# pymc-devs/pymc

Measured on AMD Instinct MI355X. Metric: effective samples/sec (and leapfrog steps/sec), 10k-param hierarchical logistic regression, one NUTS chain per GPU, higher is better.
Workload: dtype f64

## Files before the change

pymc_amd/csrc/engine.hip:

```cpp
#include <hip/hip_runtime.h>

#include <algorithm>
#include <atomic>
#include <chrono>
#include <cmath>
#include <cstdio>
#include <cstdlib>
#include <cstring>
#include <mutex>
#include <thread>
#include <utility>
#include <ctime>
#include <string>
#include <vector>

#include "kernels.h"
#include "small_kernel.h"
#include "mixture_kernel.h"
#include "nuts_mi355.h"
#include "pcg64_stream.h"
#include "advi.h"

static thread_local std::string g_err;

// ... 2049 lines not shown
  nuts_velocity_energy_fn hp_velocity_energy = nullptr;
  void* hp_user = nullptr;
  std::vector<double> hp_p, hp_v;
  double* kin_user_dev = nullptr;
  int full_adapt = 0, fa_mfma = 1;
  double *fa_L = nullptr, *fa_Lw = nullptr, *fa_fg_mean = nullptr, *fa_fg_raw = nullptr, *fa_bg_mean = nullptr, *fa_bg_raw = nullptr;
  double *fa_scratch = nullptr, *fa_rhs = nullptr;
  int *fa_fail = nullptr;
  double fa_fg_n = 0, fa_bg_n = 0;
  int64_t fa_previous_update = 0;
  std::vector<double> fa_initial_cov;
  double *wa_mean = nullptr, *wa_m2 = nullptr, *wb_mean = nullptr, *wb_m2 = nullptr;
  bool fg_is_a = true;
  double fg_count = 0, bg_count = 0;
  std::vector<double> initial_mean, initial_diag;
  int64_t n_samples = 0, adaptation_window = 101;
  bool window_switched = false;
  DualAvg da{};
  bool tune = true;
  int64_t iter_count = 0, divergences = 0;
  double step_size = 0;
  double* stage_dev = nullptr;
  double* stage_host = nullptr;
  double* out_dev = nullptr;
  double* out_dev2 = nullptr;
  bool small = false;
  int small_lds_slots = 0;
  int small_one_wave = 1;
  int group_wide = 0;
  double* out_host = nullptr;
  HostStatus* st_dev = nullptr;
  HostStatus* st_host = nullptr;
  int seq = 0;
  std::vector<double> div_source, div_dest;
  bool cache_ok = false;
  std::vector<double> last_q;
  double last_logp = 0.0;
  DrawOut* do_dev = nullptr;
  DrawOut* do_host = nullptr;
  DrawOutMapped* dom_host = nullptr;
  DrawOutMapped* dom_dev = nullptr;
  unsigned dom_seq = 0;
  double* kin_part = nullptr;
  int64_t cache_epoch = -1;
  int fold_ctl = 1;
  CtlJob pend{}; bool pend_valid = false;
  bool defer_last_ctl = false; int xfold = 1;
  int next_dir = 0; bool pre_done = false; int xpre = 1;
  bool edge_pair = false;
  ArenaDev shA{};
  EdgePlan ep;
  int spec_max = 10, last_depth = 0;
  int pipe_draws = 1;
  int logs_done = 0, logs_total = 0;
  double* many_in_host = nullptr; double* many_in_dev = nullptr; char* many_out_host = nullptr; char* many_out_dev = nullptr;
  size_t many_in_cap = 0, many_out_cap = 0;
  double t_begin = 0, t_loop = 0, t_wait = 0, t_finish = 0, t_post = 0;
  double tm_pre = 0, tm_start = 0, tm_tree = 0, tm_record = 0, tm_host = 0, tm_post = 0;
  int64_t tm_draws = 0, tm_batches = 0;
  int64_t leapfrogs = 0;
  int n_uni_cap = 0;
  template <typename T>
  T* keep(T* p) { owned.push_back((void*)p); return p; }
};

extern "C" void nuts_chain_config_default(nuts_chain_config* c) {
  std::memset(c, 0, sizeof(*c));
  c->step_scale = 0.25; c->Emax = 1000; c->target_accept = 0.8; c->gamma = 0.05; c->k = 0.75; c->t0 = 10;
  c->adapt_step_size = 1; c->max_treedepth = 10; c->early_max_treedepth = 8;
  c->potential = NUTS_POT_DIAG_ADAPT; c->initial_weight = 0; c->adaptation_window = 101; c->discard_window = 50;
  c->exp_alpha = 0.02; c->exp_stop_adaptation = INFINITY; c->exp_use_grads = 0;
  c->adaptation_window_multiplier = 1; c->early_update = 0;
}

static void fa_factor(nuts_chain* c, const double* raw, double denom) {
  const int n = c->n;
  hipStream_t s = c->m->stream;
  const dim3 g2((n + 255) / 256, n);
  hipLaunchKernelGGL(k_fa_cov, g2, dim3(256), 0, s, n, raw, denom, c->dense_C, c->fa_Lw, c->fa_fail);
  const int nb = (n + FA_NB - 1) / FA_NB;
  for (int k = 0; k < nb; ++k) {
    hipLaunchKernelGGL(k_chol_panel, dim3(nb - k), dim3(256), 0, s, n, c->fa_Lw, k, c->fa_fail);
    const int m = nb - k - 1;
    if (m > 0) hipLaunchKernelGGL(k_chol_update, dim3(m * (m + 1) / 2), dim3(256), 0, s, n, c->fa_Lw, k, nb, c->fa_mfma);
  }
  hipLaunchKernelGGL(k_fa_commit, dim3(1024), dim3(256), 0, s, (int64_t)n * n, c->fa_Lw, c->fa_L, c->fa_fail, c->fa_fail + 1);
}
static void fa_random(nuts_chain* c, const double* z_dev, double* p_out) {
  const int n = c->n;
  hipStream_t s = c->m->stream;
  hipMemcpyAsync(c->fa_rhs, z_dev, n * sizeof(double), hipMemcpyDeviceToDevice, s);
  const int nb = (n + FA_NB - 1) / FA_NB;
  for (int b = nb - 1; b >= 0; --b)
    hipLaunchKernelGGL(k_trsv_block, dim3(std::max(1, (b * FA_NB + 255) / 256)), dim3(256), 0, s, n, c->fa_L, c->fa_rhs, p_out, b);
}
static int fa_reset(nuts_chain* c) {
  const int n = c->n;
  const size_t nn = (size_t)n * n;
  const double w = c->cfg.initial_weight;
  std::vector<double> raw(nn);
  for (size_t e = 0; e < nn; ++e) raw[e] = c->fa_initial_cov[e] * w;
  HIPCHK(hipMemcpy(c->fa_fg_raw, raw.data(), nn * sizeof(double), hipMemcpyHostToDevice));
  HIPCHK(hipMemcpy(c->fa_fg_mean, c->initial_mean.data(), n * sizeof(double), hipMemcpyHostToDevice));
  HIPCHK(hipMemset(c->fa_bg_raw, 0, nn * sizeof(double)));
  HIPCHK(hipMemset(c->fa_bg_mean, 0, n * sizeof(double)));
  HIPCHK(hipMemset(c->fa_fail, 0, 2 * sizeof(int)));
// ... 51 lines not shown
    c->fg_count = w; c->bg_count = 0;
  }
  if (c->full_adapt) { const int rc = fa_reset(c); if (rc) return rc; }
  if (c->cfg.potential == NUTS_POT_DIAG_ADAPT_EXP) {
    HIPCHK(hipMemset(c->wa_mean, 0, n * sizeof(double))); HIPCHK(hipMemset(c->wa_m2, 0, n * sizeof(double)));
    HIPCHK(hipMemset(c->wb_mean, 0, n * sizeof(double))); HIPCHK(hipMemset(c->wb_m2, 0, n * sizeof(double)));
  }
  c->n_samples = 0;
  return NUTS_OK;
}

extern "C" nuts_chain* nuts_chain_create(nuts_model* m, const nuts_chain_config* cfg) {
  if (!m || !cfg) { g_err = "null argument"; return nullptr; }
  if (cfg->potential < NUTS_POT_DIAG_ADAPT || cfg->potential > NUTS_POT_HOST) { g_err = "unknown potential kind"; return nullptr;
  }
  if (cfg->potential == NUTS_POT_FULL && (!cfg->dense_cov || !cfg->dense_rand)) { g_err = "dense potential needs dense_cov and dense_rand"; return nullptr; }
  if (cfg->potential == NUTS_POT_FULL_ADAPT && !cfg->dense_cov) { g_err = "NUTS_POT_FULL_ADAPT needs dense_cov (the initial covariance)"; return nullptr; }
  if (cfg->max_treedepth < 1 || cfg->max_treedepth > MAX_LEVELS - 1) { g_err = "max_treedepth out of range (1..11)"; return nullptr; }
  if ((cfg->potential == NUTS_POT_FULL || cfg->potential == NUTS_POT_FULL_ADAPT || cfg->potential == NUTS_POT_HOST) && m->md.lg.ga) {
    g_err = "a dense mass matrix needs the span-partitioned row pass: create the model with NUTS_ROWS_NO_GROUP_ALIGNED";
    return nullptr;
  }
  auto* c = new nuts_chain();
  c->m = m; c->cfg = *cfg; c->n = m->md.n;
  m->n_chains++;
  const int n = c->n;
  c->initial_mean.assign(n, 0.0);
  c->initial_diag.assign(n, 1.0);
  if (cfg->initial_mean) c->initial_mean.assign(cfg->initial_mean, cfg->initial_mean + n);
  if (cfg->initial_diag) c->initial_diag.assign(cfg->initial_diag, cfg->initial_diag + n);
  else if (cfg->potential == NUTS_POT_DIAG_ADAPT) c->cfg.initial_weight = 1;
  c->cfg.initial_mean = nullptr; c->cfg.initial_diag = nullptr;
  c->host_pot = cfg->potential == NUTS_POT_HOST;
  c->dense = cfg->potential == NUTS_POT_FULL || cfg->potential == NUTS_POT_FULL_ADAPT || c->host_pot;
  c->full_adapt = cfg->potential == NUTS_POT_FULL_ADAPT;
  c->fa_mfma = env_int("NUTS_FA_MFMA", 1);
  if (c->cfg.fa_update_window < 1) c->cfg.fa_update_window = 1;
  if (c->dense) c->initial_diag.assign(m->md.n, 1.0);
  c->cfg.dense_cov = nullptr; c->cfg.dense_rand = nullptr;
  c->adaptation_window = cfg->adaptation_window;
  ArenaDev& A = c->A;
  A.n = n;
  const int maxd = std::max(cfg->max_treedepth, cfg->early_max_treedepth);
  A.S = 1 << maxd;
  A.ept = m->ept;
  A.nblk = m->md.nblk;
  const size_t arena = (size_t)A.S * n;
  A.Q = c->keep(dev_alloc<double>(arena)); A.P = c->keep(dev_alloc<double>(arena));
  A.V = c->keep(dev_alloc<double>(arena)); A.G = c->keep(dev_alloc<double>(arena));
  A.E = c->keep(dev_alloc<double>(A.S)); A.LOGP = c->keep(dev_alloc<double>(A.S));
  A.PS = c->keep(dev_alloc<double>((size_t)MAX_LEVELS * n));
  A.PSUM = c->keep(dev_alloc<double>(n));
  c->kin_part = c->keep(dev_alloc<double>((size_t)A.nblk));
  A.ctl = c->keep(dev_alloc<Ctl>(1));
  c->var = c->keep(dev_alloc<double>(n)); c->stds = c->keep(dev_alloc<double>(n)); c->inv_stds = c->keep(dev_alloc<double>(n));
  c->wa_mean = c->keep(dev_alloc<double>(n)); c->wa_m2 = c->keep(dev_alloc<double>(n));
  c->wb_mean = c->keep(dev_alloc<double>(n)); c->wb_m2 = c->keep(dev_alloc<double>(n));
  A.var = c->var; A.inv_stds = c->inv_stds;
  A.ga_ticket = m->md.lg.ga ? m->md.lg.ga_ticket : nullptr; A.ga_nticket = m->md.lg.ga ? 2 * m->md.lg.ga_nblk : 0;
  if (c->full_adapt) {
    const size_t nn = (size_t)n * n;
    c->fa_initial_cov.assign(cfg->dense_cov, cfg->dense_cov + nn);
    c->dense_C = c->keep(dev_alloc<double>(nn));
    c->fa_L = c->keep(dev_alloc<double>(nn)); c->fa_Lw = c->keep(dev_alloc<double>(nn));
    c->fa_fg_raw = c->keep(dev_alloc<double>(nn)); c->fa_bg_raw = c->keep(dev_alloc<double>(nn));
    c->fa_fg_mean = c->keep(dev_alloc<double>(n)); c->fa_bg_mean = c->keep(dev_alloc<double>(n));
    c->fa_scratch = c->keep(dev_alloc<double>(4 * (size_t)n)); c->fa_rhs = c->keep(dev_alloc<double>(n));
    c->fa_fail = c->keep(dev_alloc<int>(2));
    c->mv_grid = (n + (256 / WAVE) - 1) / (256 / WAVE);
  } else if (c->host_pot) {
    c->hp_p.assign(n, 0.0); c->hp_v.assign(n, 0.0);
    c->kin_user_dev = c->keep(dev_alloc<double>(1));
    A.kin_user = c->kin_user_dev;
  } else if (c->dense) {
    c->dense_C = c->keep(dev_upload(cfg->dense_cov, (size_t)n * n));
    c->dense_W = c->keep(dev_upload(cfg->dense_rand, (size_t)n * n));
    c->mv_grid = (n + (256 / WAVE) - 1) / (256 / WAVE);
  }
  c->n_uni_cap = (1 << maxd) + 2 * maxd + 16;
  c->stage_dev = c->keep(dev_alloc<double>(2 * (size_t)n + 2 * (size_t)c->n_uni_cap));
  c->out_dev = c->keep(dev_alloc<double>(2 * (size_t)n));
  c->out_dev2 = c->keep(dev_alloc<double>(2 * (size_t)n + 2));
  c->fold_ctl = env_int("NUTS_FOLD_CTL", 1) != 0 && !(m->md.has_mvn && m->md.mv.winv);
  c->spec_max = env_int("NUTS_SPEC_MAX", 10);
  c->xfold = env_int("NUTS_XFOLD", 1);
  c->edge_pair = m->ep_ok && env_int("NUTS_EDGE_PAIR", 1) != 0 && !c->dense && !c->host_pot && !m->md.has_mvn && !m->explicit_pre &&
                 m->md.lean_ok && c->fold_ctl && c->xfold;
  if (c->edge_pair) {
    c->shA = A;
    c->shA.S = 2;
    c->shA.Q = c->keep(dev_alloc<double>(2 * (size_t)n)); c->shA.P = c->keep(dev_alloc<double>(2 * (size_t)n));
    c->shA.V = c->keep(dev_alloc<double>(2 * (size_t)n)); c->shA.G = c->keep(dev_alloc<double>(2 * (size_t)n));
    if (!c->shA.Q || !c->shA.P || !c->shA.V || !c->shA.G) { (void)hipGetLastError(); c->edge_pair = false; }
    c->ep.ring = std::max(1, std::min(GA_RING_LEAVES, env_int("NUTS_EDGE_PAIR_RING", GA_RING_LEAVES)));
  }
  c->pipe_draws = env_int("NUTS_PIPE_DRAWS", 1) != 0;
  c->xpre = env_int("NUTS_XPRE", 1);
  c->small_lds_slots = env_int("NUTS_SMALL_LDS", 1) == 0 ? -1 : env_int("NUTS_SMALL_LDS_SLOTS", 0);
  c->small_one_wave = env_int("NUTS_SMALL_ONE_WAVE", 1);
  c->group_wide = env_int("NUTS_GROUP_WIDE", 0);
  const bool glm_small = m->md.has_glm && env_int("NUTS_GLM_SMALL", 1) != 0 && m->md.glm.Xt && !m->md.glm.beta_buf && m->md.glm.off_beta >= 0 && m->md.n_derived == 0 && n <= 256;
  c->small = env_int("NUTS_SMALL_KERNEL", 1) != 0 && n <= SMALL_MAX_N && m->ept == 1 && !m->md.has_logit && !m->md.has_mvn && !m->md.has_mix &&
             (!m->md.has_glm || glm_small) &&
             m->md.n_lins == 0 && m->factor_elems <= SMALL_MAX_ELEMS && !c->dense;
  c->do_dev = c->keep(dev_alloc<DrawOut>(1));
  A.uniforms = c->stage_dev + 2 * (size_t)n;
  A.log_uniforms = A.uniforms + c->n_uni_cap;
  for (void* p : c->owned)
    if (!p) { g_err = "device allocation failed (trajectory arena needs 4*2^max_treedepth*n*8 bytes)"; nuts_chain_destroy(c); return nullptr; }
  if (hipHostMalloc((void**)&c->stage_host, (2 * (size_t)n + 2 * (size_t)c->n_uni_cap) * sizeof(double), hipHostMallocDefault) != hipSuccess ||
      hipHostMalloc((void**)&c->out_host, 2 * (size_t)n * sizeof(double), hipHostMallocDefault) != hipSuccess ||
      hipHostMalloc((void**)&c->st_host, sizeof(HostStatus), hipHostMallocMapped) != hipSuccess ||
      hipHostGetDevicePointer((void**)&c->st_dev, c->st_host, 0) != hipSuccess ||
      hipHostMalloc((void**)&c->do_host, sizeof(DrawOut), hipHostMallocDefault) != hipSuccess ||
      hipHostMalloc((void**)&c->dom_host, DOM_RING * sizeof(DrawOutMapped), hipHostMallocMapped) != hipSuccess ||
      hipHostGetDevicePointer((void**)&c->dom_dev, c->dom_host, 0) != hipSuccess) {
    g_err = "pinned host allocation failed"; nuts_chain_destroy(c); return nullptr;
  }
  hipMemset(A.ctl, 0, sizeof(Ctl));
  std::memset(c->st_host, 0, sizeof(HostStatus));
  std::memset(c->dom_host, 0, DOM_RING * sizeof(DrawOutMapped));
  c->step_size = cfg->step_scale / std::pow((double)n, 0.25);
  c->da = DualAvg{c->step_size, cfg->target_accept, cfg->gamma, cfg->k, cfg->t0, 0, 0, 0, 0, 1};
  c->da.reset();
  if (potential_reset(c) != NUTS_OK) { nuts_chain_destroy(c); return nullptr; }
  return c;
}

extern "C" void nuts_chain_destroy(nuts_chain* c) {
  if (!c) return;
  if (c->m) hipStreamSynchronize(c->m->stream);
  if (c->m && c->m->group) group_remove_model(c->m->group, c->m);
  if (c->m) c->m->n_chains--;
  for (void* p : c->owned) if (p) hipFree(p);
  if (c->stage_host) hipHostFree(c->stage_host);
  if (c->out_host) hipHostFree(c->out_host);
  if (c->st_host) hipHostFree(c->st_host);
  if (c->do_host) hipHostFree(c->do_host);
  if (c->dom_host) hipHostFree(c->dom_host);
  if (c->many_in_host) hipHostFree(c->many_in_host);
  if (c->many_out_host) hipHostFree(c->many_out_host);
  if (c->many_in_dev) hipFree(c->many_in_dev);
  if (c->many_out_dev) hipFree(c->many_out_dev);
  delete c;
}

static void group_remove_model(nuts_group* g, nuts_model* m) {
  if (!g || !m || m->group != g) return;
  hipStreamSynchronize(g->stream);
  std::lock_guard<std::mutex> lk(g->mu);
  for (int i = 0; i < GRP_MAXC; ++i)
    if (g->member[i] == m) { g->member[i] = nullptr; g->n--; g->konst_set[i] = false; if (i < GAL_MAXC) g->gal_konst_set[i] = false; }
  if (m->g_active) { g->nactive--; m->g_active = false; }
  m->group = nullptr;
  m->stream = m->own_stream;
}

extern "C" nuts_group* nuts_group_create(void) {
  nuts_group* g = new nuts_group();
  if (hipStreamCreateWithFlags(&g->stream, hipStreamNonBlocking) != hipSuccess) { g_err = "nuts_group_create: no stream"; delete g; return nullptr; }
  return g;
}

extern "C" int nuts_group_add(nuts_group* g, nuts_chain* c) {
  if (!g || !c || !c->m) return NUTS_E_ARG;
  nuts_model* m = c->m;
  const MvnDev& mv = m->md.mv;
  if (m->group) { g_err = "nuts_group_add: the chain's model already belongs to a group"; return NUTS_E_ARG; }
  if (m->n_chains != 1) { g_err = "nuts_group_add: a member model carries exactly one chain (its launch parity and records are the chain's)"; return NUTS_E_ARG; }
  const RowsDev& lg = m->md.lg;
  const bool is_mvn = m->md.has_mvn && (mv.aligned == 4 || mv.aligned == 8);
  const bool is_rows = m->md.has_logit && !m->md.has_mvn && lg.ga && lg.ga_naux == 0 && lg.D == 8 && m->ga_struct_ok == 1;
// ... 424 lines not shown
  const int* abort_flag = mode == MODE_TREE ? &A.ctl->aborted : nullptr;
  const int t = gm.edge + gm.dir * (j + 1), src = gm.edge + gm.dir * j;
  const int64_t d_o = (int64_t)(t & (A.S - 1)) * A.n, so = (int64_t)(src & (A.S - 1)) * A.n;
  HostStatus* const st = mode == MODE_TREE ? c->st_dev : (HostStatus*)nullptr;
  io.lean = m->md.lean_ok && !c->dense && (!io.explicit_pre || m->md.n_deferred == 0);
  const bool foldable = c->fold_ctl && (mode == MODE_TREE || (mode == MODE_SIMPLE && n_simple > 0));
  const bool last = mode == MODE_TREE ? j + 1 == (1 << d) : j + 1 == n_simple;
  if (io.lean && foldable) {
    if (io.explicit_pre) {
      const bool al_xpre = m->md.mv.aligned && mode == MODE_TREE && c->xpre;
      if (j == 0 && !(al_xpre && c->pre_done)) hipLaunchKernelGGL(k_leaf_pre, dim3(A.nblk), dim3(VEC_THREADS), 0, s, A, io, j);
      if (j == 0) c->pre_done = false;
      io.pre_next = last ? 0 : 1;
      if (last && al_xpre && c->defer_last_ctl && c->next_dir != 0) {
        io.pre_next = c->next_dir == gm.dir ? 1 : 3;
        c->pre_done = true;
      }
    }
    const bool deferrable = (io.explicit_pre ? m->md.mv.aligned != 0 : m->md.lg.ga != 0) && mode == MODE_TREE;
    CtlJob* job = (deferrable && j == 0 && c->pend_valid) ? &c->pend : nullptr;
    if (job && !io.explicit_pre) job->src_prev = job->io.dir == io.dir;
    launch_dense(m, A, io, j, (j > 0 || job) ? 1 : 0, d, c->cfg.Emax, max_depth, st, job);
    if (job) c->pend_valid = false;
    launch_vector(m, A, io, j, d);
    if (last) {
      if (deferrable && c->defer_last_ctl) { c->pend = CtlJob{io, j, d, seq, false}; c->pend_valid = true; }
      else launch_control_lean(m, A, io, j, d, c->cfg.Emax, max_depth, st, seq);
    }
    c->leapfrogs++;
    return;
  }
  if (io.explicit_pre) hipLaunchKernelGGL(k_leaf_pre, dim3(A.nblk), dim3(VEC_THREADS), 0, s, A, io, j);
  if (c->dense)
    dense_velocity(c, A.P + d_o, A.V + d_o, A.Q + so, A.Q + d_o, gm.eps, abort_flag, VEL_ONLY);
  launch_dense(m, A, io, j, 0, d, c->cfg.Emax, max_depth, st);
  launch_vector(m, A, io, j, d);
  if (io.lean) launch_control_lean(m, A, io, j, d, c->cfg.Emax, max_depth, st, seq);
  else if (m->has_prog) hipLaunchKernelGGL(k_control<true>, dim3(1), dim3(VEC_THREADS), 0, s, m->md, A, io, j, d, c->cfg.Emax, max_depth, st, seq);
  else hipLaunchKernelGGL(k_control<false>, dim3(1), dim3(VEC_THREADS), 0, s, m->md, A, io, j, d, c->cfg.Emax, max_depth, st, seq);
  if (c->dense) {
    dense_velocity(c, A.P + d_o, A.V + d_o, nullptr, nullptr, 0.0, abort_flag, VEL_LEAF);
    const dim3 grid(m->md.nblk);
    switch (m->ept) {
      case 1: hipLaunchKernelGGL(k_tree_vec<1>, grid, dim3(VEC_THREADS), 0, s, m->md, A, io, j, d); break;
      case 4: hipLaunchKernelGGL(k_tree_vec<4>, grid, dim3(VEC_THREADS), 0, s, m->md, A, io, j, d); break;
      default: hipLaunchKernelGGL(k_tree_vec<16>, grid, dim3(VEC_THREADS), 0, s, m->md, A, io, j, d); break;
    }
    hipLaunchKernelGGL(k_tree_ctl, dim3(1), dim3(VEC_THREADS), 0, s, m->md, A, io, j, d, c->cfg.Emax, max_depth,
                       mode == MODE_TREE ? c->st_dev : (HostStatus*)nullptr, seq);
  }
  c->leapfrogs++;
}

static int run_tree(nuts_chain* c, const double* uniforms, double step_size, int max_depth, unsigned* flags_out, bool* exhausted_out,
                    int* cursor_out = nullptr) {
  int rc = NUTS_OK;
  bool exhausted = true;
  GroupTreeScope lockstep(c->dense || c->host_pot ? nullptr : c->m);
  unsigned flags = 0;
  Geometry gm{uniforms[0] < 0.5 ? 1 : -1, 0, 0, 0, 0.0};
  gm.eps = gm.dir > 0 ? step_size : -step_size;
  auto next_geometry = [&](const Geometry& g, int d, int dir) {
    Geometry r = g;
    if (g.dir > 0) r.right += 1 << d; else r.left -= 1 << d;
    r.dir = dir;
    r.edge = dir > 0 ? r.right : r.left;
    r.eps = dir > 0 ? step_size : -step_size;
    return r;
  };
  const int spec = c->host_pot ? 0 : std::min(c->spec_max, c->last_depth - 1);
  const bool pairing = c->edge_pair && !c->m->group && !c->host_pot && !c->dense;
  int turns = 0;
  int ep_replays_in[32] = {};
  int prev_dir = 0;
  bool ep_bad = false;
  c->ep.reset();
  c->m->ep_launch.kind = EP_PLAIN;
  auto enqueue_doubling = [&](const Geometry& g, int d) {
    const int nleaf = 1 << d;
    ensure_logs(c, (2 << d) + d + 1);
    const int seq = ++c->seq;
    c->defer_last_ctl = c->xfold && c->fold_ctl && d + 1 < max_depth && d + 1 <= spec;
    c->next_dir = c->defer_last_ctl ? (uniforms[(2 << d) + d] < 0.5 ? 1 : -1) : 0;
    if (pairing) c->ep.begin(d, g.dir, std::min(spec, max_depth - 1), [&](int e) { return uniforms[(1 << e) + e - 1] < 0.5 ? 1 : -1; });
    for (int j = 0; j < nleaf; ++j) {
      if (pairing) {
        nuts_model::EpLaunch& el = c->m->ep_launch;
        int k = 0;
        el.kind = c->ep.leaf(g.dir, &el.slot, &k);
        if (el.kind == EP_REPLAY) ++ep_replays_in[std::min(d, 31)];
        if (el.kind == EP_REPLAY && k != j) { g_err = "internal error: edge pairing replays a leaf out of order"; ep_bad = true; el.kind = EP_PLAIN; }
        if (el.kind == EP_PAIRED) {
          const int od = -g.dir;
          EvalIO sio{};
          sio.mode = MODE_SIMPLE; sio.lean = 1;
          sio.dir = od; sio.edge = od > 0 ? g.right : g.left; sio.left = g.left; sio.right = g.right;
          sio.eps = od > 0 ? step_size : -step_size;
          el.sio = sio; el.sj = k; el.sA = c->shA;
          el.first = k == 0;
          el.sfold = k > 0 ? GA_FOLD_SRC : (j == 0 && d > 0 && prev_dir == od ? GA_FOLD_SRC : 0);
        }
      }
      enqueue_leaf(c, g, j, d, MODE_TREE, max_depth, j + 1 == nleaf ? seq : 0);
    }
    prev_dir = g.dir;
    c->defer_last_ctl = false;
    return seq;
  };
  c->pre_done = false;
  c->pend_valid = false;
  auto flush_pending = [&](int seq_waited) {
    if (!c->pend_valid || c->pend.seq != seq_waited) return;
    const CtlJob& p = c->pend;
    launch_control_lean(c->m, c->A, p.io, p.j, p.d, c->cfg.Emax, max_depth, c->st_dev, p.seq);
    c->pend_valid = false;
  };
  Geometry ahead{};
  int ahead_seq = 0;
  int seq = enqueue_doubling(gm, 0);
  int depth_done = 0;
  for (int d = 0; d < max_depth; ++d) {
    if (d + 1 < max_depth && d + 1 <= spec) {
      ahead = next_geometry(gm, d, uniforms[(2 << d) + d] < 0.5 ? 1 : -1);
      ahead_seq = enqueue_doubling(ahead, d + 1);
    } else ahead_seq = 0;
    flush_pending(seq);
    if (c->cb_err) return host_pot_error(c);
    const auto tw0 = clk::now();
    rc = wait_status(c, seq, &flags, cursor_out);
    c->t_wait += secs(tw0, clk::now());
    if (rc) return rc;
    depth_done = d + 1;
    if (flags & ST_BAD_ENERGY) break;
    if (flags & (ST_DIVERGING | ST_TURNING)) { exhausted = false; break; }
    if (d + 1 >= max_depth) break;
    const int dir = (flags & ST_DIR_POS) ? 1 : -1;
    turns += dir != gm.dir;
    if (ahead_seq) {
      if (ahead.dir != dir) { g_err = "internal error: look-ahead mispredicted the direction of a doubling"; return NUTS_E_HIP; }
      gm = ahead; seq = ahead_seq;
    } else {
      gm = next_geometry(gm, d, dir);
      seq = enqueue_doubling(gm, d + 1);
    }
  }
  c->last_depth = depth_done;
  c->pend_valid = false;
  if (depth_done >= 4) c->m->ep_turns = std::max(c->m->ep_turns, turns);
  c->m->ep_ring_full = c->ep.ring_full;
  if (pairing) {
    c->m->ep_dropped += c->ep.n;
    for (int d = depth_done; d < 32; ++d) c->m->ep_dropped += ep_replays_in[d];
  }
  if (ep_bad) return NUTS_E_HIP;
  *flags_out = flags;
  *exhausted_out = exhausted;
  return NUTS_OK;
}

static void launch_small(nuts_chain* c, const ArenaDev& A, const SmallDrawArgs& a) {
#define SMALL_LAUNCH(NT, P) hipLaunchKernelGGL((k_small_draw<NT, P>), dim3(1), dim3(NT), 0, c->m->stream, c->m->md, A, a)
  const bool hp = c->m->has_prog;
  if (c->n <= WAVE && c->small_one_wave && !c->m->md.has_glm) { if (hp) SMALL_LAUNCH(64, true); else SMALL_LAUNCH(64, false); }
  else if (c->n <= 256) { if (hp) SMALL_LAUNCH(256, true); else SMALL_LAUNCH(256, false); }
  else if (c->n <= 512) { if (hp) SMALL_LAUNCH(512, true); else SMALL_LAUNCH(512, false); }
  else { if (hp) SMALL_LAUNCH(1024, true); else SMALL_LAUNCH(1024, false); }
#undef SMALL_LAUNCH
}

static int finish_draw_host(nuts_chain* c, const DrawOut& o, bool adapt, bool exhausted, const double* result_dev, int64_t evals,
                            double perf_start, double perf_diff, double cpu_diff, nuts_draw_stats* stats) {
  c->da.update(std::exp(o.log_accept_sum) / o.n_proposals, adapt);
  int rc = potential_update(c, result_dev, result_dev + c->n);
  if (rc) return rc;
  if (o.diverging) { rc = read_divergence_points(c, o.div_t); if (rc) return rc; }
  if (!c->tune) c->divergences += o.diverging != 0;
  c->iter_count += 1;
  fill_draw_stats(c, o, exhausted, evals, perf_start, perf_diff, cpu_diff, stats);
  return NUTS_OK;
}

static SmallDrawArgs small_draw_args(const nuts_chain* c, bool cached, const DrawPlan& plan) {
  SmallDrawArgs a{};
  a.q_src = cached ? c->out_dev2 : nullptr; a.g_src = cached ? c->out_dev2 + c->n : nullptr; a.cached_logp = c->last_logp;
  a.step_size = plan.step_size; a.Emax = c->cfg.Emax; a.max_depth = plan.max_depth;
  a.worst_uniforms = plan.need_uni;
  a.q_out = c->out_dev; a.g_out = c->out_dev + c->n; a.st = nullptr; a.seq = 0; a.lds_slots = c->small_lds_slots;
  return a;
}

static int draw_one_small(nuts_chain* c, const double* q0, const double* normals, const double* uniforms, const DrawPlan& plan,
                          bool* exhausted, const double** result_dev) {
  const int n = c->n;
  hipStream_t s = c->m->stream;
  ArenaDev& A = c->A;
  const bool cached = start_cached(c, q0);
  std::memcpy(c->stage_host, q0, n * sizeof(double));
  std::memcpy(c->stage_host + n, normals, n * sizeof(double));
  std::memcpy(c->stage_host + 2 * n, uniforms, plan.need_uni * sizeof(double));
  HIPCHK(hipMemcpyAsync(c->stage_dev, c->stage_host, (2 * (size_t)n + plan.need_uni) * sizeof(double), hipMemcpyHostToDevice, s));
  if (!cached) HIPCHK(hipMemcpyAsync(A.Q, c->stage_dev, n * sizeof(double), hipMemcpyDeviceToDevice, s));
  SmallDrawArgs a = small_draw_args(c, cached, plan);
  a.normals = c->stage_dev + n;
  a.n_draws = 1; a.n_uniforms = plan.need_uni;
  a.trace_q = nullptr; a.out = c->do_dev; a.n_done = nullptr;
  launch_small(c, A, a);
  std::swap(c->out_dev, c->out_dev2);
// ... 69 lines not shown
  double* const h_q = c->many_in_host;
  double* const h_norm = h_q + n;
  double* const h_u = h_norm + (size_t)K * n;
  double* const h_lu = h_u + U;
  std::memcpy(h_q, q0, n * sizeof(double));
  std::memcpy(h_norm, normals, (size_t)K * n * sizeof(double));
  std::memcpy(h_u, uniforms, U * sizeof(double));
  for (size_t i = 0; i < U; ++i) h_lu[i] = std::log(h_u[i]);
  HIPCHK(hipMemcpyAsync(c->many_in_dev, c->many_in_host, in_doubles * sizeof(double), hipMemcpyHostToDevice, s));
  const double* const d_norm = c->many_in_dev + n;
  const double* const d_u = d_norm + (size_t)K * n;
  const double* const d_lu = d_u + U;
  double* const trace_dev = reinterpret_cast<double*>(c->many_out_dev);
  if (!cached0) {
    HIPCHK(hipMemcpyAsync(A.Q, c->many_in_dev, n * sizeof(double), hipMemcpyDeviceToDevice, s));
    model_enqueue_plain(c->m, A.Q, A.G, A.LOGP);
  }
  const double* const save_u = A.uniforms; const double* const save_lu = A.log_uniforms;
  const int save_done = c->logs_done, save_total = c->logs_total;
  c->logs_done = c->logs_total = 1 << 30;
  int done = 0;
  size_t consumed = 0;
  const int fgrid = std::max(1, std::min(256, (n + VEC_THREADS - 1) / VEC_THREADS));
  c->tm_pre += secs(tm0, clk::now()); c->tm_batches++;
  const bool pipe = !c->tune && !c->full_adapt && c->pipe_draws;
  struct Pending {
    bool valid = false; int k = 0; unsigned seq = 0; bool exhausted = false, adapt = false; size_t consumed_after = 0; int cursor = 0;
    double perf_start = 0.0, wall = 0.0, cpu = 0.0;
  } pend;
  auto enqueue_start = [&](int k, const DrawPlan& plan, size_t at, bool from_prev) {
    A.uniforms = d_u + at; A.log_uniforms = d_lu + at;
    return enqueue_draw_start(c, d_norm + (size_t)k * n, false, from_prev, plan.step_size, 0, plan.max_depth, k > 0 ? (const DrawOut*)c->do_dev : nullptr);
  };
  auto complete = [&](const Pending& p, bool* diverged) -> int {
    const auto tb = clk::now();
    DrawOutMapped* slot = c->dom_host + (p.seq % DOM_RING);
    unsigned long long seen = 0;
    int r = wait_seq(c, &slot->seq, 0, p.seq, "k_draw_finish ended without publishing its record", &seen);
    if (r) return r;
    const DrawOut o = slot->o;
    const auto t1 = clk::now();
    c->tm_record += secs(tb, t1);
    if (o.cursor != p.cursor) { g_err = "internal error: the status word and the draw record disagree on the uniforms consumed"; return NUTS_E_HIP; }
    r = finish_draw_host(c, o, p.adapt, p.exhausted, c->out_dev, o.n_proposals + ((p.k == 0 && !cached0) ? 1 : 0), p.perf_start, p.wall, p.cpu,
                         stats + p.k);
    c->tm_host += secs(t1, clk::now()); c->tm_draws++;
    if (r) return r;
    stats[p.k].n_uniforms_consumed = (int32_t)p.consumed_after;
    c->last_logp = o.logp;
    done = p.k + 1;
    *diverged = o.diverging != 0;
    return NUTS_OK;
  };
  bool started = false;
  for (int k = 0; k < K; ++k) {
    const DrawClock dclock;
    const DrawPlan plan = plan_draw(c);
    const size_t need_uni = (size_t)plan.need_uni;
    if (!started) {
      if (U - consumed < need_uni) {
        if (k == 0) { g_err = "not enough uniforms for the worst-case tree"; rc = NUTS_E_ARG; }
        break;
      }
      rc = enqueue_start(k, plan, consumed, k > 0 || cached0);
      if (rc) break;
    }
    started = false;
    unsigned flags = 0;
    bool exhausted = true;
    int cursor = 0;
    const auto ta = clk::now();
    c->tm_start += secs(dclock.t0, ta);
    rc = run_tree(c, h_u + consumed, plan.step_size, plan.max_depth, &flags, &exhausted, &cursor);
    const auto tb = clk::now();
    c->tm_tree += secs(ta, tb);
    if (rc) break;
    if (flags & ST_BAD_ENERGY) {
      if (pend.valid) { bool dv = false; rc = complete(pend, &dv); pend.valid = false; if (rc) break; }
      rc = bad_initial_energy(c);
      break;
    }
    const unsigned seq = ++c->dom_seq;
    hipLaunchKernelGGL(k_draw_finish, dim3(fgrid), dim3(VEC_THREADS), 0, s, A, c->out_dev, c->out_dev + n, c->do_dev, trace_dev + (size_t)k * n,
                       c->dom_dev + (seq % DOM_RING), seq);
    const size_t consumed_after = consumed + (size_t)cursor;
    if (pipe && !(flags & ST_DIVERGING) && k + 1 < K && U - consumed_after >= need_uni) {
      rc = enqueue_start(k + 1, plan, consumed_after, true);
      if (rc) break;
      started = true;
    }
    Pending cur;
    cur.valid = true; cur.k = k; cur.seq = seq; cur.exhausted = exhausted; cur.adapt = plan.adapt; cur.consumed_after = consumed_after; cur.cursor = cursor;
    cur.perf_start = dclock.perf_start(); cur.wall = dclock.wall(); cur.cpu = dclock.cpu();
    bool diverged = false;
    if (pend.valid) { rc = complete(pend, &diverged); pend.valid = false; if (rc) break; }
    if (started) pend = cur;
    else { rc = complete(cur, &diverged); if (rc) break; }
    consumed = consumed_after;
    if (diverged) break;
  }
  if (pend.valid) {
    bool dv = false;
    const int r2 = complete(pend, &dv);
    pend.valid = false;
    if (!rc) rc = r2;
  }
  A.uniforms = save_u; A.log_uniforms = save_lu;
  c->logs_done = save_done; c->logs_total = save_total;
  *n_done = done;
  const auto tm1 = clk::now();
  struct PostTimer { nuts_chain* c; clk::time_point t; ~PostTimer() { c->tm_post += secs(t, clk::now()); } } post_timer{c, tm1};
  if (done > 0) {
    HIPCHK(hipMemcpyAsync(c->many_out_host, c->many_out_dev, (size_t)done * n * sizeof(double), hipMemcpyDeviceToHost, s));
    HIPCHK(hipStreamSynchronize(s));
    HIPCHK(hipGetLastError());
    const double* trace_host = reinterpret_cast<const double*>(c->many_out_host);
    std::memcpy(q_out, trace_host, (size_t)done * n * sizeof(double));
    commit_start_cache(c, trace_host + (size_t)(done - 1) * n, c->last_logp);
  } else {
    hipStreamSynchronize(s);
  }
  if (rc && done > 0 && rc != NUTS_E_BAD_ENERGY) return rc;
  return done > 0 ? NUTS_OK : (rc ? rc : NUTS_E_ARG);
}

extern "C" int nuts_chain_draw_many(nuts_chain* c, const double* q0, const double* normals, const double* uniforms,
                                    int32_t n_uniforms, int32_t K, double* q_out, nuts_draw_stats* stats, int32_t* n_done) {
  if (!c || !q0 || !normals || !uniforms || !q_out || !stats || !n_done || K <= 0) { g_err = "null argument"; return NUTS_E_ARG; }
  if (c->host_pot) { g_err = "nuts_chain_draw_many: a host potential is consulted between draws (random, update): one nuts_chain_draw per transition"; return NUTS_E_ARG; }
  if (!c->small) return draw_many_general(c, q0, normals, uniforms, n_uniforms, K, q_out, stats, n_done);
  if (c->tune) { g_err = "nuts_chain_draw_many: the chain is still tuning (the single-launch batch has no adaptation between its draws)"; return NUTS_E_ARG; }
  const DrawClock dclock;
  const int n = c->n;
  hipStream_t s = c->m->stream;
  ArenaDev& A = c->A;
  const DrawPlan plan = plan_draw(c);
  if (n_uniforms < plan.need_uni) { g_err = "not enough uniforms for the worst-case tree"; return NUTS_E_ARG; }
  const size_t in_doubles = (size_t)n + (size_t)K * n + (size_t)n_uniforms;
  const size_t trace_bytes = (size_t)K * n * sizeof(double), outs_bytes = (size_t)K * sizeof(DrawOut);
  const size_t out_bytes = trace_bytes + outs_bytes + 16;
  int rc = ensure_many_staging(c, in_doubles, out_bytes);
  if (rc) return rc;
  const bool cached = start_cached(c, q0);
  std::memcpy(c->many_in_host, q0, n * sizeof(double));
  std::memcpy(c->many_in_host + n, normals, (size_t)K * n * sizeof(double));
  std::memcpy(c->many_in_host + n + (size_t)K * n, uniforms, (size_t)n_uniforms * sizeof(double));
  HIPCHK(hipMemcpyAsync(c->many_in_dev, c->many_in_host, in_doubles * sizeof(double), hipMemcpyHostToDevice, s));
  if (!cached) HIPCHK(hipMemcpyAsync(A.Q, c->many_in_dev, n * sizeof(double), hipMemcpyDeviceToDevice, s));
  ArenaDev Am = A;
  Am.uniforms = c->many_in_dev + n + (size_t)K * n;
  SmallDrawArgs a = small_draw_args(c, cached, plan);
  a.normals = c->many_in_dev + n;
  a.n_draws = K; a.n_uniforms = n_uniforms;
  a.trace_q = reinterpret_cast<double*>(c->many_out_dev);
  a.out = reinterpret_cast<DrawOut*>(c->many_out_dev + trace_bytes);
  a.n_done = reinterpret_cast<int*>(c->many_out_dev + trace_bytes + outs_bytes);
  launch_small(c, Am, a);
// ... 135 lines not shown
  for (int k = 0; k < 7; ++k) HIPCHK(hipMemcpy(v + (size_t)k * c->n, src[k], c->n * sizeof(double), hipMemcpyDeviceToHost));
  if (c->full_adapt) {
    const size_t n = c->n, nn = n * n;
    double* w = v + 7 * n;
    const double* mats[4] = {c->dense_C, c->fa_L, c->fa_fg_raw, c->fa_bg_raw};
    for (int k = 0; k < 4; ++k) HIPCHK(hipMemcpy(w + (size_t)k * nn, mats[k], nn * sizeof(double), hipMemcpyDeviceToHost));
    HIPCHK(hipMemcpy(w + 4 * nn, c->fa_fg_mean, n * sizeof(double), hipMemcpyDeviceToHost));
    HIPCHK(hipMemcpy(w + 4 * nn + n, c->fa_bg_mean, n * sizeof(double), hipMemcpyDeviceToHost));
  }
  return NUTS_OK;
}
extern "C" int nuts_chain_set_state(nuts_chain* c, const void* blob) {
  if (!c || !blob) return NUTS_E_ARG;
  StateHeader h;
  std::memcpy(&h, blob, sizeof(h));
  if (h.magic != STATE_MAGIC || h.n != c->n) { g_err = "sampling state does not belong to this chain (frozen fields differ)"; return NUTS_E_ARG; }
  HIPCHK(hipStreamSynchronize(c->m->stream));
  c->cache_ok = false;
  c->da = h.da; c->iter_count = h.iter_count; c->divergences = h.divergences; c->n_samples = h.n_samples;
  c->adaptation_window = h.adaptation_window; c->tune = h.tune != 0; c->fg_is_a = h.fg_is_a != 0;
  c->fg_count = h.fg_count; c->bg_count = h.bg_count;
  c->fa_previous_update = h.fa_previous_update; c->fa_fg_n = h.fa_fg_n; c->fa_bg_n = h.fa_bg_n;
  const double* v = reinterpret_cast<const double*>(static_cast<const char*>(blob) + sizeof(h));
  double* dst[7] = {c->var, c->stds, c->inv_stds, c->wa_mean, c->wa_m2, c->wb_mean, c->wb_m2};
  for (int k = 0; k < 7; ++k) HIPCHK(hipMemcpy(dst[k], v + (size_t)k * c->n, c->n * sizeof(double), hipMemcpyHostToDevice));
  if (c->full_adapt) {
    const size_t n = c->n, nn = n * n;
    const double* w = v + 7 * n;
    double* mats[4] = {c->dense_C, c->fa_L, c->fa_fg_raw, c->fa_bg_raw};
    for (int k = 0; k < 4; ++k) HIPCHK(hipMemcpy(mats[k], w + (size_t)k * nn, nn * sizeof(double), hipMemcpyHostToDevice));
    HIPCHK(hipMemcpy(c->fa_fg_mean, w + 4 * nn, n * sizeof(double), hipMemcpyHostToDevice));
    HIPCHK(hipMemcpy(c->fa_bg_mean, w + 4 * nn + n, n * sizeof(double), hipMemcpyHostToDevice));
  }
  return NUTS_OK;
}

extern "C" int nuts_chain_get_scalar(nuts_chain* c, const char* name, double* out) {
  if (!c || !name || !out) return NUTS_E_ARG;
  const std::string k(name);
  if (k == "log_step") *out = c->da.log_step;
  else if (k == "log_bar") *out = c->da.log_bar;
  else if (k == "hbar") *out = c->da.hbar;
  else if (k == "count") *out = (double)c->da.count;
  else if (k == "mu") *out = c->da.mu;
  else if (k == "iter_count") *out = (double)c->iter_count;
  else if (k == "divergences") *out = (double)c->divergences;
  else if (k == "n_samples") *out = (double)c->n_samples;
  else if (k == "adaptation_window") *out = (double)c->adaptation_window;
  else if (k == "tune") *out = c->tune;
  else if (k == "fg_count") *out = c->fg_count;
  else if (k == "bg_count") *out = c->bg_count;
  else if (k == "step_size") *out = c->step_size;
  else if (k == "leapfrogs") *out = (double)c->leapfrogs;
  else if (k == "tree_kernel" || k == "tree_launches") *out = 0.0;
  else if (k == "fa_fg_n") *out = c->fa_fg_n;
  else if (k == "fa_bg_n") *out = c->fa_bg_n;
  else if (k == "fa_previous_update") *out = (double)c->fa_previous_update;
  else if (k == "single_launch") *out = c->small ? 1.0 : 0.0;
  else if (k == "window_switched") *out = c->window_switched ? 1.0 : 0.0;
  else if (k == "t_begin") *out = c->t_begin;
  else if (k == "t_loop") *out = c->t_loop;
  else if (k == "t_wait") *out = c->t_wait;
  else if (k == "tm_pre") *out = c->tm_pre;
  else if (k == "tm_start") *out = c->tm_start;
  else if (k == "tm_tree") *out = c->tm_tree;
  else if (k == "tm_record") *out = c->tm_record;
  else if (k == "tm_host") *out = c->tm_host;
  else if (k == "tm_post") *out = c->tm_post;
  else if (k == "tm_draws") *out = (double)c->tm_draws;
  else if (k == "tm_batches") *out = (double)c->tm_batches;
  else if (k == "t_finish") *out = c->t_finish;
  else { g_err = "unknown scalar " + k; return NUTS_E_ARG; }
  return NUTS_OK;
}
extern "C" int nuts_chain_get_vector(nuts_chain* c, const char* name, double* out) {
  if (!c || !name || !out) return NUTS_E_ARG;
  const std::string k(name);
  const double* src = nullptr;
  if (k == "var") src = c->var;
  else if (k == "stds") src = c->stds;
  else if (k == "inv_stds") src = c->inv_stds;
  else if (k == "fg_mean") src = c->fg_is_a ? c->wa_mean : c->wb_mean;
  else if (k == "fg_m2") src = c->fg_is_a ? c->wa_m2 : c->wb_m2;
  else if (k == "bg_mean") src = c->fg_is_a ? c->wb_mean : c->wa_mean;
  else if (k == "bg_m2") src = c->fg_is_a ? c->wb_m2 : c->wa_m2;
  else if (k == "divergence_source" || k == "divergence_dest") {
    const std::vector<double>& v = k == "divergence_source" ? c->div_source : c->div_dest;
    if ((int)v.size() != c->n) { g_err = "no divergence recorded"; return NUTS_E_ARG; }
    std::memcpy(out, v.data(), c->n * sizeof(double));
    return NUTS_OK;
  }
  else if (c->full_adapt && (k == "fa_cov" || k == "fa_chol" || k == "fa_fg_raw" || k == "fa_bg_raw")) {
    src = k == "fa_cov" ? c->dense_C : k == "fa_chol" ? c->fa_L : k == "fa_fg_raw" ? c->fa_fg_raw : c->fa_bg_raw;
    HIPCHK(hipStreamSynchronize(c->m->stream));
    HIPCHK(hipMemcpy(out, src, (size_t)c->n * c->n * sizeof(double), hipMemcpyDeviceToHost));
    return NUTS_OK;
  }
  else if (c->full_adapt && (k == "fa_fg_mean" || k == "fa_bg_mean")) src = k == "fa_fg_mean" ? c->fa_fg_mean : c->fa_bg_mean;
  else if (k == "start_p" || k == "start_v") src = k == "start_p" ? c->A.P : c->A.V;
  else { g_err = "unknown vector " + k; return NUTS_E_ARG; }
  HIPCHK(hipStreamSynchronize(c->m->stream));
  HIPCHK(hipMemcpy(out, src, c->n * sizeof(double), hipMemcpyDeviceToHost));
  return NUTS_OK;
}

extern "C" int nuts_chain_set_dense(nuts_chain* c, const double* cov, const double* rand) {
// ... 618 lines not shown
```

pymc_amd/csrc/kernels.h:

```cpp
#pragma once
#include "model_dev.h"
#include "rows_kernel.h"

#define MAX_LEVELS 12
#define NDOT (1 + 6 * (MAX_LEVELS + 1))
#define DOT_TOP (1 + 6 * MAX_LEVELS)
#define VEC_THREADS 256
#define PART_STRIDE (PART_DOT + NDOT)

#define ROWS_BLOCK 256

#define MODE_PLAIN 0
#define MODE_TREE 1
#define MODE_SIMPLE 2

struct Ctl {
  double E0;
  double log_size, log_accept_sum, max_energy_change;
  double div_dE;
  int n_proposals, depth, left, right, proposal, cursor;
  int aborted, turning, diverging, bad_energy;
  int dir, edge;
  double eps;
  double eps_abs;
// ... 1552 lines not shown
    const double logp = A.LOGP[0];
    const double E = (A.kin_user ? *A.kin_user : 0.5 * s) - logp;
    A.E[0] = E;
    c->E0 = E;
    c->log_size = 0.0;
    c->log_accept_sum = -INFINITY;
    c->max_energy_change = 0.0;
    c->div_dE = 0.0;
    c->n_proposals = 0; c->depth = 0; c->left = 0; c->right = 0; c->proposal = 0; c->cursor = 0;
    c->turning = 0; c->diverging = 0;
    c->bad_energy = !isfinite(E);
    c->aborted = c->bad_energy;
    c->eps_abs = step_size;
    c->n_leaves_total = 0;
    c->dir = 1; c->edge = 0; c->eps = step_size;
    if (dir_forced != 0) { c->dir = dir_forced; c->eps = dir_forced > 0 ? step_size : -step_size; }
    else if (!c->aborted && max_depth > 0) ctl_next_direction(c, A.uniforms);
    if (st) publish_fields(c, st);
  }
}


struct DrawOutMapped { DrawOut o; unsigned long long seq; };

__global__ __launch_bounds__(VEC_THREADS) void k_draw_finish(ArenaDev A, double* __restrict__ q_out,
                                                             double* __restrict__ g_out, DrawOut* out,
                                                             double* __restrict__ trace_q, DrawOutMapped* mapped, unsigned seq) {
  const Ctl* c = A.ctl;
  const int prop = c->proposal;
  const int64_t po = slot_off(A, prop);
  if (blockIdx.x == 0) for (int t = threadIdx.x; t < A.ga_nticket; t += blockDim.x) A.ga_ticket[t] = 0u;
  for (int i = blockIdx.x * blockDim.x + threadIdx.x; i < A.n; i += gridDim.x * blockDim.x) {
    const double qi = A.Q[po + i];
    q_out[i] = qi;
    g_out[i] = A.G[po + i];
    if (trace_q) trace_q[i] = qi;
  }
  if (blockIdx.x == 0 && threadIdx.x == 0) {
    const int ps = prop & (A.S - 1);
    DrawOut o;
    o.energy = A.E[ps]; o.logp = A.LOGP[ps]; o.E0 = c->E0;
    o.log_accept_sum = c->log_accept_sum; o.max_energy_change = c->max_energy_change; o.div_dE = c->div_dE;
    o.depth = c->depth; o.n_proposals = c->n_proposals; o.proposal = prop; o.cursor = c->cursor;
    o.turning = c->turning; o.diverging = c->diverging; o.bad_energy = c->bad_energy; o.div_t = c->div_t;
    *out = o;
    if (mapped) {
      mapped->o = o;
      __threadfence_system();
      __hip_atomic_store(&mapped->seq, (unsigned long long)seq, __ATOMIC_RELEASE, __HIP_MEMORY_SCOPE_SYSTEM);
    }
  }
}

__global__ __launch_bounds__(VEC_THREADS) void k_potential_update(int n, const double* __restrict__ x,
                                                                  double* fg_mean, double* fg_m2, double fg_count_new,
                                                                  double* bg_mean, double* bg_m2, double bg_count_new,
                                                                  double* var, double* stds, double* inv_stds, int flags) {
  for (int i = blockIdx.x * blockDim.x + threadIdx.x; i < n; i += gridDim.x * blockDim.x) {
    double m2 = fg_m2[i];
    if (flags & 1) {
      const double xi = x[i];
      double mean = fg_mean[i];
      double od = xi - mean;
      mean += od / fg_count_new;
      m2 += od * (xi - mean);
      fg_mean[i] = mean; fg_m2[i] = m2;
      double bm = bg_mean[i], b2 = bg_m2[i];
      od = xi - bm;
      bm += od / bg_count_new;
      b2 += od * (xi - bm);
      bg_mean[i] = bm; bg_m2[i] = b2;
    }
    if (flags & 2) {
      double v = m2 / fg_count_new;
      v = fmin(fmax(v, 1e-12), 1e12);
      if (isnan(m2 / fg_count_new)) v = m2 / fg_count_new;
      const double s = sqrt(v);
      var[i] = v; stds[i] = s; inv_stds[i] = 1.0 / s;
    }
  }
}

__global__ __launch_bounds__(VEC_THREADS) void k_potential_update_exp(int n, const double* __restrict__ x, const double* __restrict__ g,
                                                                      double* ms, double* vs, double* mg, double* vg, double alpha,
                                                                      double one_m_alpha, int use_grads, double* var, double* stds,
                                                                      double* inv_stds, int flags) {
  for (int i = blockIdx.x * blockDim.x + threadIdx.x; i < n; i += gridDim.x * blockDim.x) {
    if (flags & 1) {
      ms[i] = x[i]; vs[i] = 0.0;
      if (use_grads) { mg[i] = g[i]; vg[i] = 0.0; }
    }
    if (flags & 2) {
      {
        const double delta = __dsub_rn(x[i], ms[i]);
        ms[i] = __dadd_rn(ms[i], __dmul_rn(alpha, delta));
        vs[i] = __dmul_rn(one_m_alpha, __dadd_rn(vs[i], __dmul_rn(alpha, __dmul_rn(delta, delta))));
      }
      if (use_grads) {
        const double delta = __dsub_rn(g[i], mg[i]);
        mg[i] = __dadd_rn(mg[i], __dmul_rn(alpha, delta));
        vg[i] = __dmul_rn(one_m_alpha, __dadd_rn(vg[i], __dmul_rn(alpha, __dmul_rn(delta, delta))));
      }
    }
    if (flags & 4) {
      double v;
      if (use_grads) v = __dsqrt_rn(__ddiv_rn(vs[i], vg[i]));
// ... 18 lines not shown
```

Measured before the change: 20120.

## Speculatively enqueue fused draw-finish/next-tree-start kernel before tree termination is known

Adds a k_draw_turn kernel that merges the draw-finish step (copying the proposal out and publishing DrawOut) with initialising the next tree (momentum resample, kinetic-energy reduction via a ticket, Ctl reset, first direction). The host enqueues it speculatively during each doubling, before it waits on the status. The kernel checks on the device whether the tree actually terminated and returns early otherwise. Draw completion is deferred by one more draw (older/pend) to keep the queue fuller. The aim is to remove host round-trip latency and a kernel launch between consecutive NUTS draws, at the cost of extra no-op launches and more complex bookkeeping.

```diff
diff --git a/pymc_amd/csrc/engine.hip b/pymc_amd/csrc/engine.hip
--- a/pymc_amd/csrc/engine.hip
+++ b/pymc_amd/csrc/engine.hip
@@ -2125,6 +2125,9 @@
   EdgePlan ep;
   int spec_max = 10, last_depth = 0;
   int pipe_draws = 1;
+  int draw_turn = 1;
+  unsigned* turn_ticket = nullptr;
+  int64_t draw_turns_taken = 0, draw_turns_declined = 0, draw_turns_late = 0;
   int logs_done = 0, logs_total = 0;
   double* many_in_host = nullptr; double* many_in_dev = nullptr; char* many_out_host = nullptr; char* many_out_dev = nullptr;
   size_t many_in_cap = 0, many_out_cap = 0;
@@ -2282,6 +2285,7 @@
   A.PS = c->keep(dev_alloc<double>((size_t)MAX_LEVELS * n));
   A.PSUM = c->keep(dev_alloc<double>(n));
   c->kin_part = c->keep(dev_alloc<double>((size_t)A.nblk));
+  c->turn_ticket = c->keep(dev_alloc<unsigned>(1));
   A.ctl = c->keep(dev_alloc<Ctl>(1));
   c->var = c->keep(dev_alloc<double>(n)); c->stds = c->keep(dev_alloc<double>(n)); c->inv_stds = c->keep(dev_alloc<double>(n));
   c->wa_mean = c->keep(dev_alloc<double>(n)); c->wa_m2 = c->keep(dev_alloc<double>(n));
@@ -2325,6 +2329,7 @@
     c->ep.ring = std::max(1, std::min(GA_RING_LEAVES, env_int("NUTS_EDGE_PAIR_RING", GA_RING_LEAVES)));
   }
   c->pipe_draws = env_int("NUTS_PIPE_DRAWS", 1) != 0;
+  c->draw_turn = env_int("NUTS_DRAW_TURN", 1) != 0;
   c->xpre = env_int("NUTS_XPRE", 1);
   c->small_lds_slots = env_int("NUTS_SMALL_LDS", 1) == 0 ? -1 : env_int("NUTS_SMALL_LDS_SLOTS", 0);
   c->small_one_wave = env_int("NUTS_SMALL_ONE_WAVE", 1);
@@ -2348,6 +2353,7 @@
     g_err = "pinned host allocation failed"; nuts_chain_destroy(c); return nullptr;
   }
   hipMemset(A.ctl, 0, sizeof(Ctl));
+  hipMemset(c->turn_ticket, 0, sizeof(unsigned));
   std::memset(c->st_host, 0, sizeof(HostStatus));
   std::memset(c->dom_host, 0, DOM_RING * sizeof(DrawOutMapped));
   c->step_size = cfg->step_scale / std::pow((double)n, 0.25);
@@ -2878,8 +2884,20 @@
   c->leapfrogs++;
 }
 
+struct TurnReq {
+  bool allowed = false;
+  DrawTurn args{};
+  size_t uni_left = 0;
+  size_t need_uni = 0;
+  int (*before_wait)(void*) = nullptr; void* ctx = nullptr;
+  bool queued = false;
+};
+static void launch_draw_turn(nuts_chain* c, const DrawTurn& t) {
+  hipLaunchKernelGGL(k_draw_turn, dim3(c->A.nblk), dim3(VEC_THREADS), 0, c->m->stream, c->A, t);
+}
+
 static int run_tree(nuts_chain* c, const double* uniforms, double step_size, int max_depth, unsigned* flags_out, bool* exhausted_out,
-                    int* cursor_out = nullptr) {
+                    int* cursor_out = nullptr, TurnReq* turn = nullptr) {
   int rc = NUTS_OK;
   bool exhausted = true;
   GroupTreeScope lockstep(c->dense || c->host_pot ? nullptr : c->m);
@@ -2943,6 +2961,7 @@
   };
   Geometry ahead{};
   int ahead_seq = 0;
+  int turn_behind = -1;
   int seq = enqueue_doubling(gm, 0);
   int depth_done = 0;
   for (int d = 0; d < max_depth; ++d) {
@@ -2952,6 +2971,13 @@
     } else ahead_seq = 0;
     flush_pending(seq);
     if (c->cb_err) return host_pot_error(c);
+    if (turn && d == 0 && turn->before_wait) { rc = turn->before_wait(turn->ctx); if (rc) return rc; }
+    if (turn && turn->allowed && ahead_seq == 0 && turn->uni_left >= (size_t)draw_turn_bound(d) + turn->need_uni) {
+      DrawTurn t = turn->args;
+      t.d = d;
+      launch_draw_turn(c, t);
+      turn_behind = d;
+    }
     const auto tw0 = clk::now();
     rc = wait_status(c, seq, &flags, cursor_out);
     c->t_wait += secs(tw0, clk::now());
@@ -2960,6 +2986,7 @@
     if (flags & ST_BAD_ENERGY) break;
     if (flags & (ST_DIVERGING | ST_TURNING)) { exhausted = false; break; }
     if (d + 1 >= max_depth) break;
+    if (turn_behind == d) c->draw_turns_declined++;
     const int dir = (flags & ST_DIR_POS) ? 1 : -1;
     turns += dir != gm.dir;
     if (ahead_seq) {
@@ -2979,6 +3006,7 @@
     for (int d = depth_done; d < 32; ++d) c->m->ep_dropped += ep_replays_in[d];
   }
   if (ep_bad) return NUTS_E_HIP;
+  if (turn) turn->queued = turn_behind >= 0 && turn_behind == depth_done - 1;
   *flags_out = flags;
   *exhausted_out = exhausted;
   return NUTS_OK;
@@ -3154,6 +3182,25 @@
     *diverged = o.diverging != 0;
     return NUTS_OK;
   };
+  const bool turn_ok = pipe && c->draw_turn && !c->dense && !c->host_pot && !c->m->group;
+  Pending older;
+  auto turn_args = [&](int k, const DrawPlan& plan, size_t at, unsigned seq) {
+    DrawTurn t{};
+    t.normals = d_norm + (size_t)(k + 1) * n;
+    t.q_out = c->out_dev; t.g_out = c->out_dev + n; t.trace_q = trace_dev + (size_t)k * n;
+    t.out = c->do_dev; t.mapped = c->dom_dev + (seq % DOM_RING); t.seq = seq;
+    t.kin_part = c->kin_part; t.ticket = c->turn_ticket;
+    t.uni_base = d_u; t.consumed = (long long)at;
+    t.step_size = plan.step_size; t.max_depth = plan.max_depth; t.d = -1; t.st = c->st_dev;
+    return t;
+  };
+  auto complete_older = [&]() -> int {
+    if (!older.valid) return NUTS_OK;
+    bool dv = false;
+    older.valid = false;
+    return complete(older, &dv);
+  };
+  using CompleteOlder = decltype(complete_older);
   bool started = false;
   for (int k = 0; k < K; ++k) {
     const DrawClock dclock;
@@ -3173,38 +3220,69 @@
     int cursor = 0;
     const auto ta = clk::now();
     c->tm_start += secs(dclock.t0, ta);
-    rc = run_tree(c, h_u + consumed, plan.step_size, plan.max_depth, &flags, &exhausted, &cursor);
+    TurnReq treq;
+    if (turn_ok) {
+      treq.allowed = k + 1 < K;
+      treq.args = turn_args(k, plan, consumed, c->dom_seq + 1);
+      treq.uni_left = U - consumed; treq.need_uni = need_uni;
+      treq.before_wait = [](void* f) { return (*static_cast<CompleteOlder*>(f))(); };
+      treq.ctx = &complete_older;
+    }
+    rc = run_tree(c, h_u + consumed, plan.step_size, plan.max_depth, &flags, &exhausted, &cursor, turn_ok ? &treq : nullptr);
     const auto tb = clk::now();
     c->tm_tree += secs(ta, tb);
     if (rc) break;
     if (flags & ST_BAD_ENERGY) {
-      if (pend.valid) { bool dv = false; rc = complete(pend, &dv); pend.valid = false; if (rc) break; }
+      rc = complete_older();
+      if (pend.valid) { bool dv = false; const int r2 = complete(pend, &dv); pend.valid = false; if (!rc) rc = r2; }
+      if (rc) break;
       rc = bad_initial_energy(c);
       break;
     }
     const unsigned seq = ++c->dom_seq;
-    hipLaunchKernelGGL(k_draw_finish, dim3(fgrid), dim3(VEC_THREADS), 0, s, A, c->out_dev, c->out_dev + n, c->do_dev, trace_dev + (size_t)k * n,
-                       c->dom_dev + (seq % DOM_RING), seq);
     const size_t consumed_after = consumed + (size_t)cursor;
-    if (pipe && !(flags & ST_DIVERGING) && k + 1 < K && U - consumed_after >= need_uni) {
-      rc = enqueue_start(k + 1, plan, consumed_after, true);
-      if (rc) break;
+    const bool next_ok = pipe && !(flags & ST_DIVERGING) && k + 1 < K && U - consumed_after >= need_uni;
+    if (turn_ok && treq.queued && !(flags & ST_DIVERGING)) {
+      if (!next_ok) { g_err = "internal error: a draw turn-over was queued ahead of uniforms that cannot cover the next tree"; rc = NUTS_E_HIP; break; }
+      c->draw_turns_taken++;
       started = true;
-    }
+    } else if (turn_ok && next_ok) {
+      launch_draw_turn(c, turn_args(k, plan, consumed, seq));
+      c->draw_turns_late++;
+      started = true;
+    } else {
+      hipLaunchKernelGGL(k_draw_finish, dim3(fgrid), dim3(VEC_THREADS), 0, s, A, c->out_dev, c->out_dev + n, c->do_dev, trace_dev + (size_t)k * n,
+                         c->dom_dev + (seq % DOM_RING), seq);
+      if (next_ok) {
+        rc = enqueue_start(k + 1, plan, consumed_after, true);
+        if (rc) break;
+        started = true;
+      }
+    }
+    if (started) { A.uniforms = d_u + consumed_after; A.log_uniforms = d_lu + consumed_after; }
     Pending cur;
     cur.valid = true; cur.k = k; cur.seq = seq; cur.exhausted = exhausted; cur.adapt = plan.adapt; cur.consumed_after = consumed_after; cur.cursor = cursor;
     cur.perf_start = dclock.perf_start(); cur.wall = dclock.wall(); cur.cpu = dclock.cpu();
     bool diverged = false;
-    if (pend.valid) { rc = complete(pend, &diverged); pend.valid = false; if (rc) break; }
-    if (started) pend = cur;
-    else { rc = complete(cur, &diverged); if (rc) break; }
+    if (turn_ok && started) {
+      rc = complete_older();
+      if (rc) break;
+      older = pend; pend = cur;
+    } else {
+      rc = complete_older();
+      if (rc) break;
+      if (pend.valid) { rc = complete(pend, &diverged); pend.valid = false; if (rc) break; }
+      if (started) pend = cur;
+      else { rc = complete(cur, &diverged); if (rc) break; }
+    }
     consumed = consumed_after;
     if (diverged) break;
   }
-  if (pend.valid) {
+  for (Pending* p : {&older, &pend}) {
+    if (!p->valid) continue;
     bool dv = false;
-    const int r2 = complete(pend, &dv);
-    pend.valid = false;
+    const int r2 = complete(*p, &dv);
+    p->valid = false;
     if (!rc) rc = r2;
   }
   A.uniforms = save_u; A.log_uniforms = save_lu;
@@ -3446,6 +3524,9 @@
   else if (k == "bg_count") *out = c->bg_count;
   else if (k == "step_size") *out = c->step_size;
   else if (k == "leapfrogs") *out = (double)c->leapfrogs;
+  else if (k == "draw_turns_taken") *out = (double)c->draw_turns_taken;
+  else if (k == "draw_turns_declined") *out = (double)c->draw_turns_declined;
+  else if (k == "draw_turns_late") *out = (double)c->draw_turns_late;
   else if (k == "tree_kernel" || k == "tree_launches") *out = 0.0;
   else if (k == "fa_fg_n") *out = c->fa_fg_n;
   else if (k == "fa_bg_n") *out = c->fa_bg_n;
diff --git a/pymc_amd/csrc/kernels.h b/pymc_amd/csrc/kernels.h
--- a/pymc_amd/csrc/kernels.h
+++ b/pymc_amd/csrc/kernels.h
@@ -1628,6 +1628,94 @@
   }
 }
 
+struct DrawTurn {
+  const double* normals;
+  double *q_out, *g_out, *trace_q;
+  DrawOut* out; DrawOutMapped* mapped; unsigned seq;
+  double* kin_part;
+  unsigned* ticket;
+  const double* uni_base; long long consumed;
+  double step_size; int max_depth;
+  int d;
+  HostStatus* st;
+};
+
+__host__ __device__ __forceinline__ bool draw_turn_taken(int diverging, int bad_energy, int turning, int d, int max_depth) {
+  return !diverging && !bad_energy && (turning || d + 1 >= max_depth);
+}
+__host__ __device__ __forceinline__ int draw_turn_bound(int d) { return (2 << d) + d + 1; }
+
+__global__ __launch_bounds__(VEC_THREADS) void k_draw_turn(ArenaDev A, DrawTurn T) {
+  __shared__ double sm[VEC_THREADS / WAVE];
+  Ctl* c = A.ctl;
+  if (T.d >= 0 && !draw_turn_taken(c->diverging, c->bad_energy, c->turning, T.d, T.max_depth)) return;
+  const int prop = c->proposal;
+  const int64_t po = slot_off(A, prop);
+  if (blockIdx.x == 0) for (int t = threadIdx.x; t < A.ga_nticket; t += VEC_THREADS) A.ga_ticket[t] = 0u;
+  double kin = 0.0;
+  const int base = blockIdx.x * VEC_THREADS * A.ept;
+  for (int e = 0; e < A.ept; ++e) {
+    const int i = base + e * VEC_THREADS + threadIdx.x;
+    if (i < A.n) {
+      const double qi = A.Q[po + i], gi = A.G[po + i];
+      T.q_out[i] = qi; T.g_out[i] = gi;
+      if (T.trace_q) T.trace_q[i] = qi;
+      const double p = T.normals[i] * A.inv_stds[i];
+      const double v = A.var[i] * p;
+      A.P[i] = p; A.V[i] = v;
+      A.PSUM[i] = p;
+      A.Q[i] = qi; A.G[i] = gi;
+      kin = fma(p, v, kin);
+    }
+  }
+  const double tot = block_sum<false>(kin, sm);
+  if (threadIdx.x != 0) return;
+  st_agent(T.kin_part + blockIdx.x, tot);
+  asm volatile("s_waitcnt vmcnt(0)" ::: "memory");
+  const unsigned old = __hip_atomic_fetch_add(T.ticket, 1u, __ATOMIC_RELAXED, __HIP_MEMORY_SCOPE_AGENT);
+  if (old + 1 != gridDim.x) return;
+  __hip_atomic_store(T.ticket, 0u, __ATOMIC_RELAXED, __HIP_MEMORY_SCOPE_AGENT);
+  __builtin_amdgcn_fence(__ATOMIC_ACQUIRE, "agent");
+  const int ps = prop & (A.S - 1);
+  DrawOut o;
+  o.energy = A.E[ps]; o.logp = A.LOGP[ps]; o.E0 = c->E0;
+  o.log_accept_sum = c->log_accept_sum; o.max_energy_change = c->max_energy_change; o.div_dE = c->div_dE;
+  o.depth = c->depth; o.n_proposals = c->n_proposals; o.proposal = prop; o.cursor = c->cursor;
+  o.turning = c->turning; o.diverging = c->diverging; o.bad_energy = c->bad_energy; o.div_t = c->div_t;
+  *T.out = o;
+  if (T.mapped) {
+    T.mapped->o = o;
+    __threadfence_system();
+    __hip_atomic_store(&T.mapped->seq, (unsigned long long)T.seq, __ATOMIC_RELEASE, __HIP_MEMORY_SCOPE_SYSTEM);
+  }
+  double s = 0.0;
+  for (int b0 = 0; b0 < A.nblk; b0 += 8) {
+    double v[8];
+#pragma unroll
+    for (int u = 0; u < 8; ++u) v[u] = ld_agent(T.kin_part + min(b0 + u, A.nblk - 1));
+#pragma unroll
+    for (int u = 0; u < 8; ++u) if (b0 + u < A.nblk) s += v[u];
+  }
+  const double* uniforms = T.uni_base + T.consumed + o.cursor;
+  A.LOGP[0] = o.logp;
+  const double E = (A.kin_user ? *A.kin_user : 0.5 * s) - o.logp;
+  A.E[0] = E;
+  c->E0 = E;
+  c->log_size = 0.0;
+  c->log_accept_sum = -INFINITY;
+  c->max_energy_change = 0.0;
+  c->div_dE = 0.0;
+  c->n_proposals = 0; c->depth = 0; c->left = 0; c->right = 0; c->proposal = 0; c->cursor = 0;
+  c->turning = 0; c->diverging = 0;
+  c->bad_energy = !isfinite(E);
+  c->aborted = c->bad_energy;
+  c->eps_abs = T.step_size;
+  c->n_leaves_total = 0;
+  c->dir = 1; c->edge = 0; c->eps = T.step_size;
+  if (!c->aborted && T.max_depth > 0) ctl_next_direction(c, uniforms);
+  if (T.st) publish_fields(c, T.st);
+}
+
 __global__ __launch_bounds__(VEC_THREADS) void k_potential_update(int n, const double* __restrict__ x,
                                                                   double* fg_mean, double* fg_m2, double fg_count_new,
                                                                   double* bg_mean, double* bg_m2, double bg_count_new,
```

Measured after the change: 20140, median of 5. No clear change (+0.1%).
